# inksci/TRPO

Measured on AMD Instinct MI355X. Metric: TRPO updates/sec (10-iter CG + linesearch) at N states; FVP GB/s vs HBM peak, higher is better.
Workload: dtype fp32 (f16x3 split); 1 GPU; C4: 8M states, obs 128, 256x256 tanh MLP, 18 actions; full update = discount+standardise+pg+10 CG+shs FVP+line search+final losses; n_states=8000000, obs_dim=128, n_actions=18, num_params=103442, cg_iters=10, parallelism=dp1 (row shards, RCCL all-reduce of [P] FVP/grad + loss scalars)

## Files before the change

### trpo_amd/csrc/engine.cpp

```cpp
#include "../../include/trpo_engine.h"
#include "abi_util.h"
#include "common.h"
#include "kernels.h"

#include <hip/hip_runtime.h>
#include <rccl/rccl.h>

#include <algorithm>
#include <cmath>
#include <cstddef>
#include <cstdio>
#include <cstdlib>
#include <cstring>
#include <map>
#include <memory>
#include <stdexcept>
#include <string>
#include <type_traits>
#include <vector>

using namespace trpo;

using namespace trpo_abi;

// ... 1542 lines not shown
        a.am_a0 = am_ds(1);
        Scope sp(this, "pg_bwdwg_l1");
        launch_rbwd0(a, stream);
        check_launch();
        continue;
      }
      RowGemmArgs a = row_args(w[l], wp[l]);
      a.nseg = 1;
      a.seg[0] = bwd_seg(l, kW, DS[l], am_ds(l));
      a.epi = RowEpi::kPgBwd;
      a.ea.H = H[l];
      a.ea.out0 = DS[l - 1];
      a.ea.amax0 = am_ds(l - 1);
      a.ea.ldo = wp[l];
      Scope sp(this, "pg_bwd", l);
      launch_rowgemm(a, stream);
      check_launch();
    }
    for (int l = r0f ? 1 : 0; l < (have_ds ? L - 1 : L); ++l)
      wgrad_layer(l, 1, WSeg{act_in(l), DS[l], wp[l], wp[l + 1], l == 0 ? am_x() : nullptr, am_ds(l)}, WSeg{}, 0,
                  nullptr, "pg_wgrad");
    reduce_grad(g, nullptr);
  }

  void fvp(const float* v, float* out, const int* skip, int* defer = nullptr) {
    if (defer) *defer = 0;
    reprepare_if_path_changed();
    prepare();
    cache.rd_written();
    cache.slabs_written();
    if (use_fused16()) {
      fvp_fused16(v, out, skip, defer && !multi_rank() && cg_fused_reduce_ok(P) ? defer : nullptr);
      return;
    }
    if (use_fused()) {
      fvp_fused(v, out, skip);
      return;
    }
    if (use_chain()) {
      fvp_chain(v, out, skip);
      return;
    }
    {
      PackArgs pa = pack_args(WF, &WB, 1);
      launch_pack(pa, v, 1, skip, stream);
      check_launch();
    }
    ensure_w3();
    const bool gs = gauss();
    split_parts(false, true, false, !gs, cur_set(), skip, "split_v");
    am_reset(am_rh(0), L);
    am_reset(am_rd(0), L);
    const bool tail = use_tail();
    const int Lf = tail ? L - 1 : L;
    int l_first = 0;
    const bool rh1p = use_rh1_planes();
    if (use_rfwd01()) {
      {
        Scope sp(this, "fvp_rfwd_img");
        launch_rfwd01_img(theta, v, offW[0], offW[1], w[0], am_v(0), am_w(1), am_v(1), rf_img, skip, stream);
        check_launch();
      }
      Rfwd01Args ra{};
      ra.n = n;
      ra.obs = w[0];
      ra.ldh = wp[1];
      ra.ldz = wp[2];
      ra.Xh = Xh;
      ra.Xl = Xl;
      ra.x_mpad = x_mpad;
      ra.eX = pl_e;
      ra.H1 = H[1];
      ra.c0 = v + offb[0];
      ra.c1 = v + offb[1];
      ra.V0 = v + offW[0];
      ra.RH1 = RH[1];
      ra.RZ2 = RH[2];
      ra.img = rf_img;
      ra.am_v0 = am_v(0);
      ra.am_w1 = am_w(1);
      ra.am_v1 = am_v(1);
      ra.am_rh1 = am_rh(1);
      ra.am_rz2 = am_rh(2);
      if (rh1p) ra.e_rh1 = pl_e + 2;
      ra.skip = skip;
      Scope sp(this, "fvp_rfwd01");
      launch_rfwd01(ra, num_cus, stream);
      check_launch();
      l_first = 2;
    }
    for (int l = l_first; l < Lf; ++l) {
      RowGemmArgs a = row_args(w[l + 1], wp[l + 1]);
      if (l == 0) {
        a.nseg = 1;
        a.seg[0] = fwd_seg(0, kV, X, am_x(), cur_set());
        if (planes_l0()) attach_x_planes(a.seg[0], V0b);
      } else {
        a.nseg = 2;
        a.seg[0] = fwd_seg(l, kW, RH[l], am_rh(l), cur_set());
        a.seg[1] = fwd_seg(l, kV, H[l], nullptr, cur_set());
      }
      a.skip = skip;
      a.ea.bias = v + offb[l];
      a.ea.ldo = wp[l + 1];
      if (l < L - 1) {
        a.epi = (tail && l == L - 2) ? RowEpi::kRZ : RowEpi::kRHidden;
        a.ea.H = H[l + 1];
        a.ea.out0 = RH[l + 1];
        a.ea.amax0 = am_rh(l + 1);
      } else {
        a.epi = gs ? RowEpi::kGaussRHead : RowEpi::kRHead;
        a.ea.P = Pm;
        a.ea.logstd = gs ? logstd_of(theta) : nullptr;
        a.ea.out0 = RD[L - 1];
        a.ea.amax0 = am_rd(L - 1);
        a.ea.invN = 1.0 / (double)n_global;
      }
      Scope sp(this, "fvp_rfwd", l);
      launch_rowgemm(a, stream);
      check_launch();
    }
    if (tail) {
      const int l = L - 1;
      TailPackArgs tp{};
      tp.theta = theta;
      tp.v = v;
      tp.off_w = offW[l];
      tp.a = w[l];
      tp.b = w[l + 1];
      tp.am_w = am_w(l);
      tp.am_v = am_v(l);
      tp.out = tail_planes;
      TailArgs ta{};
      ta.rows = (int)n;
      ta.a = w[l];
      ta.b = w[l + 1];
      ta.apad = wp[l];
      ta.bpad = wp[l + 1];
      ta.RH = RH[l];
      ta.rz = 1;
      ta.H = H[l];
      ta.P = Pm;
      ta.DL = D[l];
      ta.c = v + offb[l];
      ta.WV16 = tail_planes;
      ta.WT16 = WB3[l];
      ta.VT16 = WB3[l] + 3 * plane3_b(l);
      ta.bplane = (int64_t)plane3_b(l);
      ta.am_rh = am_rh(l);
      ta.am_d = am_d(l);
      ta.am_w = am_w(l);
      ta.am_v = am_v(l);
      ta.am_out = am_rd(l - 1);
      ta.RDout = RD[l - 1];
      ta.invN = 1.0 / (double)n_global;
      ta.dst = slab_dst(l);
      ta.skip = skip;
      Scope sp(this, "fvp_tail", l);
      launch_tail_pack(tp, stream);
      launch_fvp_tail(ta, stream);
      check_launch();
    }
    const bool r0f = use_rbwd0() && Lf - 1 >= 1;
    for (int l = Lf - 1; l >= 1; --l) {
      if (l == 1 && r0f && gs) {
        RBwd0Args a = rbwd0_args(skip);
        a.nseg = 1;
        a.A0 = RD[1];
        a.am_a0 = am_rd(1);
        Scope sp(this, "fvp_rbwdwg_l1");
        launch_rbwd0(a, stream);
        check_launch();
        continue;
      }
      if (gs) {
        RowGemmArgs a = row_args(w[l], wp[l]);
        a.nseg = 1;
        a.seg[0] = bwd_seg(l, kW, RD[l], am_rd(l));
        a.skip = skip;
        a.epi = RowEpi::kPgBwd;
        a.ea.H = H[l];
        a.ea.out0 = RD[l - 1];
        a.ea.amax0 = am_rd(l - 1);
        a.ea.ldo = wp[l];
        Scope sp(this, "fvp_rbwd", l);
        launch_rowgemm(a, stream);
        check_launch();
        continue;
      }
      if (l == 1 && r0f) {
        RBwd0Args a = rbwd0_args(skip);
        a.nseg = 2;
        a.A0 = RD[1];
        a.A1 = D[1];
        if (cache.d1_plane) {
          a.A1h = D1h;
          a.a1_mpad = cache.d1_mpad;
          a.eA1p = pl_e + 1;
          if (cache.d1_tiled) a.eA1t = eD1t;
        }
        a.am_a0 = am_rd(1);
        a.am_a1 = am_d(1);
        a.E = E[0];
        a.RH = RH[1];
        if (rh1p) a.RHp = rh1_planes();
        Scope sp(this, "fvp_rbwdwg_l1");
        launch_rbwd0(a, stream);
        check_launch();
        continue;
      }
      RowGemmArgs a = row_args(w[l], wp[l]);
      a.nseg = 2;
      a.seg[0] = bwd_seg(l, kW, RD[l], am_rd(l));
      a.seg[1] = bwd_seg(l, kV, D[l], am_d(l));
      a.skip = skip;
      a.epi = RowEpi::kRBwd;
      a.ea.H = H[l];
      a.ea.E = E[l - 1];
      a.ea.RH = RH[l];
      a.ea.out0 = RD[l - 1];
      a.ea.amax0 = am_rd(l - 1);
      a.ea.ldo = wp[l];
      Scope sp(this, "fvp_rbwd", l);
      launch_rowgemm(a, stream);
      check_launch();
    }
    if (gs) {
      for (int l = r0f ? 1 : 0; l < L; ++l)
        wgrad_layer(l, 1, WSeg{act_in(l), RD[l], wp[l], wp[l + 1], l == 0 ? am_x() : nullptr, am_rd(l)}, WSeg{}, 0, skip,
                    "fvp_wgrad");
      reduce_grad(out, skip, 0, v + (P - w[L]));
      return;
    }
    fvp_wgrads(r0f ? 1 : 0, Lf, skip, rh1p);
    reduce_grad(out, skip);
  }

  ChainArgs chain_args(const ImageSet& is, const float* v, const int* skip) const {
    ChainArgs ca{};
    ca.n = (int)n;
    ca.L = L;
    for (int l = 0; l <= L; ++l) {
      ca.w[l] = w[l];
      ca.ld[l] = wp[l];
    }
    ca.X = X;
    for (int l = 0; l < L; ++l) {
      ca.H[l] = H[l];
      ca.RH[l] = RH[l];
      ca.D[l] = D[l];
      ca.E[l] = E[l];
      ca.RD[l] = RD[l];
      ca.offb[l] = offb[l];
    }
    ca.P = Pm;
    ca.v = v;
    ca.img = is.img;
    ca.tab = is.tab;
    ca.nchunks = is.nchunks;
    ca.invN = 1.0 / (double)n_global;
    ca.skip = skip;
    return ca;
  }
  void chain_w_images(const float* v) {
    if (cache.chain_w_valid) return;
    Scope sp(this, "fvp_img_w");
    launch_chain_img(chain_set.jobs, theta, v, 0, nullptr, stream);
    check_launch();
    cache.chain_w_valid = true;
  }
  void chain_images(const float* v, const int* skip) {
    chain_w_images(v);
    Scope sp(this, "fvp_img_v");
    launch_chain_img(chain_set.jobs, theta, v, 1, skip, stream);
    check_launch();
  }

  void fvp_fused(const float* v, float* out, const int* skip) {
    chain_images(v, skip);
    const int variant = g_options.fused == 1 ? 1 : 2;
    const int rb = fused_fvp_states_per_group(variant);
    FusedArgs fa{};
    fa.c = chain_args(chain_set, v, skip);
    fa.slab = slab;
    fa.slab_stride = slab_stride;
    for (int l = 0; l < L; ++l) fa.offW[l] = offW[l];
    fa.ngroups = (int)((n + rb - 1) / rb);
    const int per_cu = variant == 2 ? 2 : 1;
    const int grid =
        (int)std::max<int64_t>(1, std::min<int64_t>({(int64_t)fa.ngroups, (int64_t)S, (int64_t)num_cus * per_cu}));
    {
      Scope sp(this, "fvp_fused");
      launch_fvp_fused(fa, grid, variant, stream);
      check_launch();
    }
    reduce_grad(out, skip, grid);
  }

  Fused16Args fused16_args(const float* v, const int* skip, int& grid) {
    const int rb = fused16_states_per_group();
    Fused16Args fa{};
    fa.f.c = chain_args(f16_set, v, skip);
    fa.f.slab = slab;
    fa.f.slab_stride = slab_stride;
    for (int l = 0; l < L; ++l) fa.f.offW[l] = offW[l];
    fa.f.ngroups = (int)((n + rb - 1) / rb);
// ... 1373 lines not shown
```

### trpo_amd/csrc/kernels.h

```cpp
#pragma once
#include <hip/hip_runtime.h>
#include <cstdint>

namespace trpo {

struct Options {
  int split_mfma;
  int split_wg;
  int chain;
  int split_f16;
  int split_min_k;
  int graphs;
  int tail;
  int fused;
  int low_seg;
  int planes;
  int rbwd0;
  int hbwd2;
  int head_fwd;
  int splits;
  int pg_splits;
  int ls_fused;
  int cg_fuse_reduce;
  int cg_p_img;
  int rfwd01;
  int fwd01;
  int rh1_planes;
  int rbwd0_bdma;
};

constexpr int kAmaxSub = 256, kAmaxStride = 32, kAmaxSlot = kAmaxSub * kAmaxStride;

__host__ __device__ inline int f16_scale_exp(float m) {
  if (!(m > 0.0f) || !(m < 3.0e38f)) return 0;
  int q = 0;
  (void)frexpf(m, &q);
  int e = 12 - q;
  return e < -100 ? -100 : (e > 100 ? 100 : e);
}
extern Options g_options;
int* option_slot(const char* name);

struct GemmSeg {
  const float* A;
  const float* B;
  int lda, ldb, K;
  const uint16_t* B3 = nullptr;
  int ldk = 0, plane = 0;
  const unsigned* amaxA = nullptr;
  const unsigned* amaxB = nullptr;
  const uint16_t* Ah = nullptr;
  const uint16_t* Al = nullptr;
  int ldp = 0, mpad = 0;
  const int* eAp = nullptr;
  const uint16_t* Bb = nullptr;
};

enum class RowEpi : int {
  kTanh = 0,
  kRHidden = 1,
  kPrepBwd = 2,
  kPgBwd = 3,
  kRBwd = 4,
  kPrepHead = 5,
  kLossHead = 6,
  kRHead = 7,
  kRelu = 8,
  kReluBwd = 9,
  kPrepBwdE = 10,
  kRZ = 11,
  kGaussPrepHead = 12,
  kGaussLossHead = 13,
  kGaussRHead = 14,
};
constexpr int kMaxHeadTiles = 4;
constexpr bool epi_is_gauss(int e) { return e >= (int)RowEpi::kGaussPrepHead && e <= (int)RowEpi::kGaussRHead; }
constexpr bool epi_is_head(int e) {
  return (e >= (int)RowEpi::kPrepHead && e <= (int)RowEpi::kRHead) || epi_is_gauss(e);
}

struct RowEpiArgs {
  const float* bias;
  const float* H;
  const float* E;
  const float* RH;
  float* out0;
  float* out1;
  float* out2;
  int ldo;
  const float* P;
  const float* old;
  const int* act;
  const float* adv;
  double* rowterms;
  double invN;
  unsigned* amax0 = nullptr;
  unsigned* amax1 = nullptr;
  unsigned* amax2 = nullptr;
  const float* actf = nullptr;
  const float* logstd = nullptr;
  const float* logstd0 = nullptr;
};

struct RowGemmArgs {
  int M, N, Npad;
  int nseg;
  GemmSeg seg[2];
  const int* skip;
  RowEpi epi;
  RowEpiArgs ea;
  int f16 = 0;
  int low_seg = 0;
};

void launch_rowgemm(const RowGemmArgs& a, hipStream_t s);
void launch_rowgemm_planes(const RowGemmArgs& a, hipStream_t s);
void launch_split_planes(const float* A, int M, int Mpad, int K, int lda, uint16_t* hi, uint16_t* lo, int ldp,
                         const unsigned* amax, int* e_out, hipStream_t s);
void launch_block_planes(const uint16_t* src, int P, int R, int ld, uint16_t* dst, hipStream_t s);
bool rowgemm_uses_split(int Npad, RowEpi epi);

struct SplitJob {
  const float* B;
  uint16_t* B3;
  int K, Npad, ldb, ldk;
  const unsigned* amax = nullptr;
};
constexpr int kMaxSplitJobs = 16;
struct SplitArgs {
  int n;
  SplitJob job[kMaxSplitJobs];
  int f16 = 0;
};
void launch_split_b(const SplitArgs& a, const int* skip, hipStream_t s);

struct SlabDst {
  int splits = 0, rows_per_split = 0;
  float* slab = nullptr;
  int64_t slab_stride = 0;
  int64_t off_w = 0, off_b = 0;
};

struct PairPlane {
  const unsigned* hi = nullptr;
  const unsigned* lo = nullptr;
  const int* e = nullptr;
};
constexpr int kPairLd = 256;
constexpr int64_t pair_plane_dwords(int64_t rows) { return (rows + 1) / 2 * kPairLd; }

struct WSeg {
  const float* A;
  const float* B;
  int lda, ldb;
  const unsigned* amaxA = nullptr;
  const unsigned* amaxB = nullptr;
  PairPlane Ap{};
};

struct WGradArgs {
  int rows;
  int Ma, Nb;
  int Mpad, Npad;
  int nseg;
  WSeg seg[2];
  int colsum_seg;
  SlabDst dst;
  const int* skip;
  int f16 = 0;
  int low_seg = 0;
};

void launch_wgrad(const WGradArgs& a, hipStream_t s);

struct LayerPack {
  int64_t off_w;
  int a, b, apad, bpad;
  float* WF;
  float* WB;
  unsigned* amax = nullptr;
};
// ... 95 lines not shown
  void* dst;
};
struct GatherArgs {
  GatherWide wide[3];
  GatherScalar scalar[2];
  int nwide, nscalar;
  int64_t n_sub, stride;
  int64_t first;
  const float* whole_src;
  float* whole_dst;
  int64_t whole_n;
};
void launch_gather_feed(const GatherArgs& a, int num_cus, hipStream_t s);

size_t discount_workspace_bytes(int64_t n);
void launch_discount(const double* x, const uint8_t* starts, int64_t n, double gamma, double* out,
                     void* workspace, hipStream_t s);
void launch_adv_center_partials(const double* returns, const double* baseline, double* adv,
                                int64_t n, double* partials, hipStream_t s);
void launch_sum_finish(const double* partials, double* out, hipStream_t s);
void launch_adv_sq_partials(const double* adv, int64_t n, const double* global_sum, double inv_n,
                            double* partials, hipStream_t s);
void launch_adv_normalize(double* adv, float* adv32, int64_t n, const double* global_sum,
                          const double* global_sq, double inv_n, hipStream_t s);

size_t gae_workspace_bytes(int64_t n);
void launch_gae(const double* rewards, const double* values, const uint8_t* starts, const double* tail_values,
                int64_t n, double gamma, double lambda, double* adv, double* returns, void* workspace,
                hipStream_t s);

}

namespace trpo {
struct ChainArgs {
  int n, L;
  int w[kMaxLayers + 1];
  int ld[kMaxLayers + 1];
  const float* X;
  const float* H[kMaxLayers];
  float* RH[kMaxLayers];
  const float* P;
  const float* D[kMaxLayers];
  const float* E[kMaxLayers];
  float* RD[kMaxLayers];
  const float* v;
  int64_t offb[kMaxLayers];
  const void* img;
  const int* tab;
  int nchunks;
  double invN;
  const int* skip;
};

struct ChainImgJob {
  int64_t src_off, dst_off;
  int K, O, ldw, trans, kc, otp, which, pad;
};
constexpr int kMaxChainJobs = 4 * kMaxLayers;
struct ChainImgArgs {
  int n;
  ChainImgJob job[kMaxChainJobs];
  unsigned short* img;
};
int chain_max_tiles(int max_hidden);
void launch_fvp_chain(const ChainArgs& a, int otm, hipStream_t s);
void launch_chain_img(const ChainImgArgs& a, const float* theta, const float* v, int which, const int* skip,
                      hipStream_t s);

struct FusedArgs {
  ChainArgs c;
  float* slab;
  int64_t slab_stride;
  int64_t offW[kMaxLayers];
  int ngroups;
};
bool fused_fvp_eligible(int L, const int* w);
int fused_fvp_states_per_group(int variant);
void launch_fvp_fused(const FusedArgs& a, int grid, int variant, hipStream_t s);

constexpr int kFused16Jobs = 9;
struct Fused16Args {
  FusedArgs f;
  const int* img_e;
  const unsigned* am_x;
  const unsigned* am_d1;
  const unsigned* am_d2;
  const float* DS;
  const unsigned* am_ds2;
  float* D1out;
  float* E1out;
  float* E0out;
  unsigned* am_d1_out;
};
bool fused16_eligible(int L, const int* w);
int fused16_obs_chunks(int obs);
int fused16_states_per_group();
int fused16_groups_per_cu();
void launch_cg_p_img16(const ChainImgArgs& a, const float* r, const float* p_old, float* p_new, int64_t n,
                       UpdScalars* sc, const double* partials2, CGFlags* fl, int it, int* img_e, hipStream_t s);
void launch_fused16_img(const ChainImgArgs& a, const float* theta, const float* v, int which, const int* skip,
                        int* img_e, hipStream_t s);
void launch_fvp_fused16(const Fused16Args& a, int grid, hipStream_t s);
void launch_pg_fused16(const Fused16Args& a, int grid, hipStream_t s);
void launch_prep_pg_fused16(const Fused16Args& a, int grid, hipStream_t s);
struct FwdLoss16Args {
  int64_t n;
  int L = 3;
  int w[4], ld[4];
  const float* X;
  const float* theta;
  int64_t offb[3];
  const void* img;
  const int* tab;
  int nchunks;
  const int* img_e;
  const unsigned* am_x;
  const float* old;
  const int* act;
  const float* adv;
  double* rowterms;
  const int* skip;
  float* H1 = nullptr;
  float* H2 = nullptr;
  float* P = nullptr;
  float* D = nullptr;
  float* DS = nullptr;
  unsigned* am_d = nullptr;
  unsigned* am_ds = nullptr;
  double invN = 0.0;
};
void launch_fwd_loss16(const FwdLoss16Args& a, int num_cus, hipStream_t s);
}

namespace trpo {
constexpr int kTailK = 256;
struct TailArgs {
  int rows, a, b, apad, bpad;
  const float* RH;
  const float* H;
  int rz = 0;
  const float* P;
  const float* DL;
  const float* c;
  const uint16_t* WV16;
  const uint16_t* WT16;
  const uint16_t* VT16;
  int64_t bplane;
  const unsigned *am_rh, *am_d, *am_w, *am_v;
  unsigned* am_out;
  float* RDout;
  double invN;
  SlabDst dst;
  const int* skip;
};
struct TailPackArgs {
  const float* theta;
  const float* v;
  int64_t off_w;
  int a, b;
  const unsigned *am_w, *am_v;
  uint16_t* out;
};
bool tail_eligible(int apad, int bpad);

struct RBwd0Args {
  int rows;
  int K, lda;
  int N, Npad;
  int obs;
  int nseg;
  const float* A0;
  const float* A1;
  const uint16_t* A1h;
  const int* eA1t = nullptr;
  int a1_mpad;
  const int* eA1p;
  const uint16_t* B0;
  const uint16_t* B1;
  int ldk;
  int64_t plane;
  const unsigned *am_a0, *am_b0, *am_a1, *am_b1;
  const float* H;
  const float* E;
  const float* RH;
  PairPlane RHp{};
  const uint16_t* Xh;
  const uint16_t* Xl;
  int x_mpad, x_ldp;
  const int* eX;
  SlabDst dst;
  const int* skip;
  int low_seg = 0;
};
struct HeadBwd2Args {
  int rows;
  int A, Apad;
  int N, Npad;
  const float* WB;
  const float* D2;
  const float* DS2;
  const float* H;
  float* D1;
  float* DS1;
  unsigned* am_d1;
  unsigned* am_ds1;
  uint16_t* D1h = nullptr;
  int d1_mpad = 0;
  int* eD1t = nullptr;
  float* E1 = nullptr;
  SlabDst dst;
};
bool head_bwd2_eligible(int A, int Npad);
struct HeadFwdArgs {
  int64_t rows;
  int A, Apad;
  int K, Kpad;
  const float* H;
  const float* W;
  const float* bias;
  const float* old;
  const int* act;
  const float* adv;
  double* rowterms;
  double invN;
  int prep = 0;
  float* P = nullptr;
  float* D = nullptr;
  float* DS = nullptr;
  unsigned* am_d = nullptr;
  unsigned* am_ds = nullptr;
};
bool head_fwd_eligible(int A, int K);
void launch_head_fwd(const HeadFwdArgs& a, int num_cus, hipStream_t s);
void launch_head_bwd2(const HeadBwd2Args& a, int num_cus, hipStream_t s);
struct Rfwd01Args {
  int64_t n;
  int obs, ldh, ldz;
  const uint16_t *Xh, *Xl;
  int x_mpad;
  const int* eX;
  const float *H1, *c0, *c1;
  const float* V0;
  float *RH1, *RZ2;
  int* e_rh1 = nullptr;
  const uint16_t* img;
  const unsigned *am_v0, *am_w1, *am_v1;
  unsigned *am_rh1, *am_rz2;
  const int* skip;
};
struct Fwd01Args {
  int64_t n;
  int obs;
  const uint16_t *Xh, *Xl;
  int x_mpad;
  const int* eX;
  const float *b0, *b1;
  float *H1, *H2;
  const uint16_t* img;
  const unsigned *am_w0, *am_w1;
};
constexpr bool rfwd01_rows_ok(int64_t x_mpad) { return 4 * x_mpad * 64 < (int64_t(1) << 31); }
static_assert(rfwd01_rows_ok((1 << 23) - 256) && !rfwd01_rows_ok(1 << 23), "rfwd01 / fwd01 row limit");
constexpr bool pair_planes_rows_ok(int64_t x_mpad) { return rfwd01_rows_ok(x_mpad); }
bool fwd01_eligible(int L, const int* w, const int* wp);
size_t fwd01_img_bytes();
void launch_fwd01_img(const float* th, int64_t offW0, int64_t offW1, int obs, const unsigned* am_w0,
                      const unsigned* am_w1, uint16_t* img, hipStream_t s);
void launch_fwd01(const Fwd01Args& a, int num_cus, hipStream_t s);
bool rfwd01_eligible(int L, const int* w, const int* wp);
size_t rfwd01_img_bytes();
void launch_rfwd01_img(const float* theta, const float* v, int64_t offV0, int64_t offW1, int obs,
                       const unsigned* am_v0, const unsigned* am_w1, const unsigned* am_v1, uint16_t* img,
                       const int* skip, hipStream_t s);
void launch_rfwd01(const Rfwd01Args& a, int num_cus, hipStream_t s);
bool rbwd0_eligible(int obs_pad, int x_ldp, int hid_pad, int K);
void launch_rbwd0(const RBwd0Args& a, hipStream_t s);
void launch_tail_pack(const TailPackArgs& p, hipStream_t s);
void launch_fvp_tail(const TailArgs& a, hipStream_t s);
}

namespace trpo {
size_t vf_pos_workspace_bytes(int64_t n);
void launch_vf_features(const float* obs, int obs_dim, int ld_obs, const float* dist, int A, int ld_dist,
                        const uint8_t* starts, int64_t n, int64_t* lastpos, void* ws, float* feat, int Fp,
                        hipStream_t s, const int64_t* step_index = nullptr);
void launch_vf_tail_features(const float* obs, int obs_dim, const float* dist, int A, const int64_t* lengths,
                             int64_t n_paths, float* feat, int Fp, hipStream_t s);
void launch_vf_tail_scatter(const float* pred, const uint8_t* truncated, const int64_t* end_rows, int64_t n_paths,
                            int64_t n, double* tail, hipStream_t s);
struct VFPackArgs {
  int F, H1, H2, H1p, H2p;
  int64_t offW1, offW2;
  float* W1p;
  float* W2p;
  float* W2T;
};
void launch_vf_pack(const VFPackArgs& a, const float* theta, hipStream_t s);
struct VFHeadArgs {
  int64_t n;
  int H2, H2p;
  const float* Z2;
  const float* w3;
  const float* b3;
  int train;
  const float* y;
  float* dout;
// ... 121 lines not shown
```

### trpo_amd/csrc/options.cpp

```cpp
#include "kernels.h"

#include <cstdlib>
#include <cstring>

namespace trpo {
namespace {

struct OptionRow {
  const char* name;
  const char* env;
  int Options::*field;
  int dflt;
};
constexpr OptionRow kOptionRows[] = {
    {"split_mfma", "TRPO_SPLIT_MFMA", &Options::split_mfma, 5},
    {"split_wg", "TRPO_SPLIT_WG", &Options::split_wg, 1},
    {"chain", "TRPO_CHAIN", &Options::chain, 1},
    {"split_f16", "TRPO_SPLIT_F16", &Options::split_f16, 1},
    {"split_min_k", "TRPO_SPLIT_MIN_K", &Options::split_min_k, 0},
    {"graphs", "TRPO_GRAPHS", &Options::graphs, 1},
    {"tail", "TRPO_TAIL", &Options::tail, 1},
    {"fused", "TRPO_FUSED", &Options::fused, 3},
    {"low_seg", "TRPO_LOW_SEG", &Options::low_seg, 14},
    {"planes", "TRPO_PLANES", &Options::planes, 1},
    {"rbwd0", "TRPO_RBWD0", &Options::rbwd0, 1},
    {"hbwd2", "TRPO_HBWD2", &Options::hbwd2, 2},
    {"head_fwd", "TRPO_HEAD_FWD", &Options::head_fwd, 1},
    {"splits", "TRPO_SPLITS", &Options::splits, 0},
    {"pg_splits", "TRPO_PG_SPLITS", &Options::pg_splits, 0},
    {"ls_fused", "TRPO_LS_FUSED", &Options::ls_fused, 1},
    {"cg_fuse_reduce", "TRPO_CG_FUSE_REDUCE", &Options::cg_fuse_reduce, 1},
    {"cg_p_img", "TRPO_CG_P_IMG", &Options::cg_p_img, 1},
    {"rfwd01", "TRPO_RFWD01", &Options::rfwd01, 1},
    {"fwd01", "TRPO_FWD01", &Options::fwd01, 1},
    {"rh1_planes", "TRPO_RH1_PLANES", &Options::rh1_planes, 1},
    {"rbwd0_bdma", "TRPO_RBWD0_BDMA", &Options::rbwd0_bdma, 1},
};
static_assert(sizeof kOptionRows / sizeof kOptionRows[0] == sizeof(Options) / sizeof(int),
              "every field of Options needs a row");

Options options_from_env() {
  Options o{};
  for (const OptionRow& r : kOptionRows) {
    const char* e = std::getenv(r.env);
    o.*r.field = e ? std::atoi(e) : r.dflt;
  }
  return o;
}

}

Options g_options = options_from_env();

int* option_slot(const char* name) {
  for (const OptionRow& r : kOptionRows)
    if (!std::strcmp(name, r.name)) return &(g_options.*r.field);
  return nullptr;
}

}
```

### trpo_amd/csrc/tail.hip

```cpp
#include "split.h"

#include <stdexcept>

namespace trpo {
namespace {

constexpr int TR = 32;
constexpr int NW = 8;
constexpr int SLD = 36;

#ifndef TRPO_TAIL_HEAD64
#define TRPO_TAIL_HEAD64 0
#endif

__device__ __forceinline__ int sw_off(int mat, int plane, int j, int k) {
  return ((mat * 2 + plane) * 32 + j) * kTailK + (((k >> 3) ^ (j & 15)) << 3) + (k & 7);
}

__global__ void __launch_bounds__(NW * 64, 1) fvp_tail_kernel(const TailArgs A) {
  __shared__ __attribute__((aligned(16))) unsigned short sW[2 * 2 * 32 * kTailK];
  __shared__ __attribute__((aligned(16))) unsigned short sX[NW][2 * 2 * 32 * 32];
  __shared__ __attribute__((aligned(16))) float sRD[2][TR][SLD];
  __shared__ __attribute__((aligned(16))) float sD[2][TR][SLD];
  __shared__ __attribute__((aligned(16))) unsigned short sP[2 * 2 * TR * 32];
  __shared__ float sMax[2][NW];
  __shared__ float sBias[NW][64];
  __shared__ float sOut[NW];
  if (A.skip && *A.skip) return;

  const int tid = threadIdx.x, lane = tid & 63, w = tid >> 6;
  const int lr = lane & 31, lh = lane >> 5;
  const int apad = A.apad, bpad = A.bpad, b = A.b;
  const int r0 = blockIdx.x * A.dst.rows_per_split;
  const int r1 = min(A.rows, r0 + A.dst.rows_per_split);
  const int col0 = 32 * w;
  const bool wv = col0 < apad;

  const int eRH = amax_exp(A.am_rh), eD = amax_exp(A.am_d), eW = amax_exp(A.am_w), eV = amax_exp(A.am_v);
  const int eH = f16_scale_exp(1.0f);
  const float sRHf = __builtin_ldexpf(1.0f, eRH), sDf = __builtin_ldexpf(1.0f, eD), sHf = __builtin_ldexpf(1.0f, eH);

  for (int i = tid; i < 2 * 2 * 32 * (kTailK / 8); i += NW * 64) {
    const int c = i % (kTailK / 8), row = i / (kTailK / 8);
    const int j = row & 31;
    *reinterpret_cast<u16x8*>(sW + row * kTailK + ((c ^ (j & 15)) << 3)) =
        *reinterpret_cast<const u16x8*>(A.WV16 + (size_t)row * kTailK + 8 * c);
  }

  f16x8 wt[2][2], vt[2][2];
  {
    const int n = col0 + lr;
    const bool nv = n < apad;
#pragma unroll
    for (int s = 0; s < 2; ++s)
#pragma unroll
      for (int p = 0; p < 2; ++p) {
        const size_t o = (size_t)p * A.bplane + (size_t)(nv ? n : 0) * 32 + 16 * s + 8 * lh;
        const u16x8 x = *reinterpret_cast<const u16x8*>(A.WT16 + o);
        const u16x8 y = *reinterpret_cast<const u16x8*>(A.VT16 + o);
        wt[s][p] = nv ? __builtin_bit_cast(f16x8, x) : f16x8{};
        vt[s][p] = nv ? __builtin_bit_cast(f16x8, y) : f16x8{};
      }
  }
  __syncthreads();

  f32x16 G = f32x16{};
  float bsum = 0.0f;
  float mxo = 0.0f;

  auto desc = [&](const float* p, int t0, int ld) {
    const int nr = max(0, min(TR, r1 - t0));
    return __builtin_amdgcn_make_buffer_rsrc((void*)(p + (size_t)t0 * ld), 0, nr * ld * 4, 0x00020000);
  };
  const int vo_c = wv ? ((4 * lh) * apad + col0 + lr) * 4 : 0x40000000;
  const int hrow0 = ((2 * w) & 3) + 8 * ((2 * w) >> 2) + 4 * lh;
  const int vo_h = lr < bpad ? (hrow0 * bpad + lr) * 4 : 0x40000000;
  auto load_c = [&](int t0, float (&rh)[16], float (&h)[16], float (&pp)[2], float (&dd)[2]) {
    const __amdgpu_buffer_rsrc_t rRH = desc(A.RH, t0, apad), rH = desc(A.H, t0, apad);
#pragma unroll
    for (int i = 0; i < 16; ++i) {
      const int so = ((i & 3) + 8 * (i >> 2)) * apad * 4;
      rh[i] = ldbuf(rRH, vo_c, so);
      h[i] = ldbuf(rH, vo_c, so);
    }
    const __amdgpu_buffer_rsrc_t rP = desc(A.P, t0, bpad), rDL = desc(A.DL, t0, bpad);
#pragma unroll
    for (int q = 0; q < 2; ++q) {
      pp[q] = ldbuf(rP, vo_h, q * bpad * 4);
      dd[q] = ldbuf(rDL, vo_h, q * bpad * 4);
    }
  };

  float cRH[16], cH[16], cP[2], cD[2];
  if (r0 < r1) load_c(r0, cRH, cH, cP, cD);
  int par = 0;
  for (int t0 = r0; t0 < r1; t0 += TR, par ^= 1) {
    float nRH[16], nH[16], nP[2], nD[2];
    if (t0 + TR < r1) load_c(t0 + TR, nRH, nH, nP, nD);
    if (A.rz) {
#pragma unroll
      for (int i = 0; i < 16; ++i) cRH[i] = one_minus_sq(cH[i]) * cRH[i];
    }

    unsigned short* xw = sX[w];
    auto xoff = [](int mat, int plane, int k, int m) {
      return ((mat * 2 + plane) * 32 + k) * 32 + ((((m >> 2) ^ ((k >> 1) & 7))) << 2) + (m & 3);
    };
#pragma unroll
    for (int s2 = 0; s2 < 2; ++s2) {
      f16x8 hi, lo;
#pragma unroll
      for (int mat = 0; mat < 2; ++mat) {
        split8(mat == 0 ? &cRH[8 * s2] : &cH[8 * s2], mat == 0 ? sRHf : sHf, hi, lo);
        const s16x4* hp = reinterpret_cast<const s16x4*>(&hi);
        const s16x4* lp = reinterpret_cast<const s16x4*>(&lo);
#pragma unroll
        for (int half = 0; half < 2; ++half) {
          const int m = 16 * s2 + 8 * half + 4 * lh;
          *reinterpret_cast<s16x4*>(xw + xoff(mat, 0, lr, m)) = hp[half];
          *reinterpret_cast<s16x4*>(xw + xoff(mat, 1, lr, m)) = lp[half];
        }
      }
    }
    {
      const int g4 = lane >> 4, q = (lane >> 2) & 3, pp = lane & 3;
      const int mrow = 16 * (g4 & 1) + 4 * pp;
      f32x16 acc = f32x16{}, accv = f32x16{};
      auto tr8 = [&](int mat, int pl, int s2) {
        s16x8 v;
#pragma unroll
        for (int t = 0; t < 2; ++t) {
          const int k = 16 * s2 + 8 * (g4 >> 1) + 4 * t + q;
          const s16x4 r = __builtin_amdgcn_ds_read_tr16_b64_v4i16(
              (__attribute__((address_space(3))) s16x4*)(xw + xoff(mat, pl, k, mrow)));
#pragma unroll
          for (int e = 0; e < 4; ++e) v[4 * t + e] = r[e];
        }
        return __builtin_bit_cast(f16x8, v);
      };
#pragma unroll
      for (int s2 = 0; s2 < 2; ++s2) {
        const int k = col0 + 16 * s2 + 8 * lh;
        acc = mfma3(tr8(0, 0, s2), tr8(0, 1, s2), *reinterpret_cast<const f16x8*>(sW + sw_off(0, 0, lr, k)),
                    *reinterpret_cast<const f16x8*>(sW + sw_off(0, 1, lr, k)), acc);
        accv = mfma3(tr8(1, 0, s2), tr8(1, 1, s2), *reinterpret_cast<const f16x8*>(sW + sw_off(1, 0, lr, k)),
                     *reinterpret_cast<const f16x8*>(sW + sw_off(1, 1, lr, k)), accv);
      }
      const float f0 = __builtin_ldexpf(1.0f, -(eRH + eW)), f1 = __builtin_ldexpf(1.0f, -(eH + eV));
      float* rzw = reinterpret_cast<float*>(xw);
#pragma unroll
      for (int i = 0; i < 16; ++i) rzw[i * 64 + lane] = acc[i] * f0 + accv[i] * f1;
    }
    lds_barrier();

    float m = 0.0f;
    {
      const int j = lr;
      const bool real = j < b;
      const float cj = A.c[real ? j : 0];
#pragma unroll
      for (int q = 0; q < 2; ++q) {
        const int i = 2 * w + q;
        float zs = 0.0f;
#pragma unroll
        for (int u = 0; u < NW; ++u) zs += reinterpret_cast<const float*>(sX[u])[i * 64 + lane];
        const float z = zs + cj;
#if TRPO_TAIL_HEAD64
        typedef double T;
#else
        typedef float T;
#endif
        const T rz = real ? (T)z : T(0);
        const T pd = real ? (T)cP[q] : T(0);
        const T prz = sum32<TRPO_TAIL_DPP>(pd * rz);
        const T Rp = pd * (rz - prz);
        const T inv = T(1) / (pd + (T)kEps);
        const T Aa = real ? pd * inv : T(0);
        const T B = real ? (T)kEps * inv : T(0);
        const T spB = sum32<TRPO_TAIL_DPP>(pd * B);
        const T sRAB = sum32<TRPO_TAIL_DPP>(Rp * Aa * B);
        const T rd = (T)A.invN * (Rp * (B - spB) + Rp * Aa * Aa + pd * sRAB);
        const float rdf = real ? (float)rd : 0.0f;
        const int row = hrow0 + q;
        sRD[par][row][j] = rdf;
        sD[par][row][j] = real ? cD[q] : 0.0f;
        m = fmaxf(m, fabsf(rdf));
        bsum += rdf;
      }
    }
#pragma unroll
    for (int off = 32; off > 0; off >>= 1) m = fmaxf(m, __shfl_xor(m, off, 64));
    if (lane == 0) sMax[par][w] = m;
    lds_barrier();
    float mt = 0.0f;
#pragma unroll
    for (int u = 0; u < NW; ++u) mt = fmaxf(mt, sMax[par][u]);
    const int eRD = f16_scale_exp(mt);
    const float sRDf = __builtin_ldexpf(1.0f, eRD);

    auto pof = [](int mat, int pl, int row, int col) {
      return ((mat * 2 + pl) * TR + row) * 32 + ((((col >> 3) ^ ((row >> 2) & 3))) << 3) + (col & 7);
    };
    {
      const int row = 4 * w + (lane >> 4), col = 2 * (lane & 15);
#pragma unroll
      for (int mat = 0; mat < 2; ++mat) {
        const float sc = mat == 0 ? sRDf : sDf;
        const float a = (mat == 0 ? sRD[par][row][col] : sD[par][row][col]) * sc;
        const float bb = (mat == 0 ? sRD[par][row][col + 1] : sD[par][row][col + 1]) * sc;
        const u32x2 p = split2(a, bb);
        *reinterpret_cast<unsigned*>(sP + pof(mat, 0, row, col)) = p[0];
        *reinterpret_cast<unsigned*>(sP + pof(mat, 1, row, col)) = p[1];
      }
    }
    lds_barrier();

    f32x16 aRW = f32x16{}, aDV = f32x16{}, aDW = f32x16{};
#pragma unroll
    for (int s = 0; s < 2; ++s) {
      const int col = 16 * s + 8 * lh;
      const f16x8 rh_ = *reinterpret_cast<const f16x8*>(sP + pof(0, 0, lr, col));
      const f16x8 rl_ = *reinterpret_cast<const f16x8*>(sP + pof(0, 1, lr, col));
      const f16x8 dh_ = *reinterpret_cast<const f16x8*>(sP + pof(1, 0, lr, col));
      const f16x8 dl_ = *reinterpret_cast<const f16x8*>(sP + pof(1, 1, lr, col));
      aRW = mfma3(rh_, rl_, wt[s][0], wt[s][1], aRW);
      aDV = mfma3(dh_, dl_, vt[s][0], vt[s][1], aDV);
      aDW = mfma3(dh_, dl_, wt[s][0], wt[s][1], aDW);
    }
    {
      const float fRW = __builtin_ldexpf(1.0f, -(eRD + eW)), fDV = __builtin_ldexpf(1.0f, -(eD + eV));
      const float fDW = __builtin_ldexpf(1.0f, -(eD + eW));
      const __amdgpu_buffer_rsrc_t rOut = desc(A.RDout, t0, apad);
#pragma unroll
      for (int i = 0; i < 16; ++i) {
        const float rdh = aRW[i] * fRW + aDV[i] * fDV;
        const float dh = aDW[i] * fDW;
        const float h = cH[i], rh = cRH[i];
        const float e = -2.0f * dh * h;
        const float o = fmaf(e, rh, rdh * one_minus_sq(h));
        __builtin_amdgcn_raw_buffer_store_b32(__builtin_bit_cast(unsigned, o), rOut, vo_c,
                                              ((i & 3) + 8 * (i >> 2)) * apad * 4, 0);
        mxo = fmaxf(mxo, fabsf(o));
      }
    }
    {
      const int g4 = lane >> 4, q = (lane >> 2) & 3, pp = lane & 3;
      auto trb = [&](int mat, int pl, int s2) {
        s16x8 v;
#pragma unroll
        for (int t = 0; t < 2; ++t) {
          const int row = 16 * s2 + 4 * (g4 >> 1) + 8 * t + q;
          const s16x4 r = __builtin_amdgcn_ds_read_tr16_b64_v4i16(
              (__attribute__((address_space(3))) s16x4*)(sP + pof(mat, pl, row, 16 * (g4 & 1) + 4 * pp)));
#pragma unroll
          for (int e = 0; e < 4; ++e) v[4 * t + e] = r[e];
        }
        return __builtin_bit_cast(f16x8, v);
      };
      f32x16 g0 = f32x16{}, g1 = f32x16{};
#pragma unroll
      for (int s = 0; s < 2; ++s) {
        f16x8 ah, al;
        split8(&cRH[8 * s], sRHf, ah, al);
        g0 = mfma3(ah, al, trb(1, 0, s), trb(1, 1, s), g0);
        split8(&cH[8 * s], sHf, ah, al);
        g1 = mfma3(ah, al, trb(0, 0, s), trb(0, 1, s), g1);
      }
      const float fG0 = __builtin_ldexpf(1.0f, -(eRH + eD)), fG1 = __builtin_ldexpf(1.0f, -(eH + eRD));
#pragma unroll
      for (int i = 0; i < 16; ++i) G[i] += g0[i] * fG0 + g1[i] * fG1;
    }

    if (t0 + TR < r1) {
#pragma unroll
      for (int i = 0; i < 16; ++i) {
        cRH[i] = nRH[i];
        cH[i] = nH[i];
      }
#pragma unroll
      for (int q = 0; q < 2; ++q) {
        cP[q] = nP[q];
        cD[q] = nD[q];
      }
    }
  }

  float* out = A.dst.slab + (size_t)blockIdx.x * A.dst.slab_stride;
  if (lr < b) {
#pragma unroll
    for (int i = 0; i < 16; ++i) {
      const int mrow = col0 + (i & 3) + 8 * (i >> 2) + 4 * lh;
      if (mrow < A.a) out[A.dst.off_w + (int64_t)mrow * b + lr] = G[i];
    }
  }
  sBias[w][lane] = bsum;
#pragma unroll
  for (int off = 32; off > 0; off >>= 1) mxo = fmaxf(mxo, __shfl_xor(mxo, off, 64));
  if (lane == 0) sOut[w] = mxo;
  __syncthreads();
  if (tid < b) {
    float t = 0.0f;
#pragma unroll
    for (int q = 0; q < NW; ++q) t += sBias[q][tid] + sBias[q][tid + 32];
    out[A.dst.off_b + tid] = t;
  }
  if (tid == 0 && A.am_out) {
    float mm = 0.0f;
#pragma unroll
    for (int q = 0; q < NW; ++q) mm = fmaxf(mm, sOut[q]);
    if (mm > 0.0f) atomicMax(A.am_out + (blockIdx.x % kAmaxSub) * kAmaxStride, __float_as_uint(mm));
  }
}

__global__ void __launch_bounds__(256) tail_pack_kernel(const TailPackArgs P) {
  const int mat = blockIdx.y;
  const float* src = (mat == 0 ? P.theta : P.v) + P.off_w;
  const int e = amax_exp(mat == 0 ? P.am_w : P.am_v);
  const float s = __builtin_ldexpf(1.0f, e);
  const int idx = blockIdx.x * 256 + threadIdx.x;
  if (idx >= 32 * kTailK) return;
  const int j = idx / kTailK, k = idx % kTailK;
  const float x = (j < P.b && k < P.a) ? src[(size_t)k * P.b + j] * s : 0.0f;
  unsigned short hh, ll;
  split2_rn(x, hh, ll);
  P.out[((size_t)(mat * 2 + 0) * 32 + j) * kTailK + k] = hh;
  P.out[((size_t)(mat * 2 + 1) * 32 + j) * kTailK + k] = ll;
}

}

bool tail_eligible(int apad, int bpad) {
  return apad > 128 && apad <= kTailK && apad % 32 == 0 && bpad > 16 && bpad <= 32;
}

void launch_tail_pack(const TailPackArgs& p, hipStream_t s) {
  hipLaunchKernelGGL(tail_pack_kernel, dim3((32 * kTailK + 255) / 256, 2), dim3(256), 0, s, p);
}

void launch_fvp_tail(const TailArgs& a, hipStream_t s) {
  if (!tail_eligible(a.apad, a.bpad) || a.b > 32 || a.a > a.apad)
    throw std::runtime_error("fvp_tail: unsupported layer shape");
  if (a.dst.splits <= 0) return;
  if (a.dst.rows_per_split % TR) throw std::runtime_error("fvp_tail: rows_per_split % 32");
  hipLaunchKernelGGL(fvp_tail_kernel, dim3(a.dst.splits), dim3(NW * 64), 0, s, a);
}

}
```

Measured before the change: 2.547 updates/s.

## Add reduced-precision tail FVP variant selected by on-device exponent sampling

```diff
diff --git a/trpo_amd/csrc/engine.cpp b/trpo_amd/csrc/engine.cpp
--- a/trpo_amd/csrc/engine.cpp
+++ b/trpo_amd/csrc/engine.cpp
@@ -1718,6 +1718,7 @@
       ta.am_w = am_w(l);
       ta.am_v = am_v(l);
       ta.am_out = am_rd(l - 1);
+      ta.am_rdl = am_rd(l);
       ta.RDout = RD[l - 1];
       ta.invN = 1.0 / (double)n_global;
       ta.dst = slab_dst(l);
diff --git a/trpo_amd/csrc/kernels.h b/trpo_amd/csrc/kernels.h
--- a/trpo_amd/csrc/kernels.h
+++ b/trpo_amd/csrc/kernels.h
@@ -27,6 +27,7 @@
   int fwd01;
   int rh1_planes;
   int rbwd0_bdma;
+  int tail_form;
 };
 
 constexpr int kAmaxSub = 256, kAmaxStride = 32, kAmaxSlot = kAmaxSub * kAmaxStride;
@@ -428,6 +429,8 @@
   double invN;
   SlabDst dst;
   const int* skip;
+  unsigned* am_rdl = nullptr;
+  int low_seg = 0;
 };
 struct TailPackArgs {
   const float* theta;
diff --git a/trpo_amd/csrc/options.cpp b/trpo_amd/csrc/options.cpp
--- a/trpo_amd/csrc/options.cpp
+++ b/trpo_amd/csrc/options.cpp
@@ -35,6 +35,7 @@
     {"fwd01", "TRPO_FWD01", &Options::fwd01, 1},
     {"rh1_planes", "TRPO_RH1_PLANES", &Options::rh1_planes, 1},
     {"rbwd0_bdma", "TRPO_RBWD0_BDMA", &Options::rbwd0_bdma, 1},
+    {"tail_form", "TRPO_TAIL_FORM", &Options::tail_form, 1},
 };
 static_assert(sizeof kOptionRows / sizeof kOptionRows[0] == sizeof(Options) / sizeof(int),
               "every field of Options needs a row");
diff --git a/trpo_amd/csrc/tail.hip b/trpo_amd/csrc/tail.hip
--- a/trpo_amd/csrc/tail.hip
+++ b/trpo_amd/csrc/tail.hip
@@ -17,6 +17,20 @@
   return ((mat * 2 + plane) * 32 + j) * kTailK + (((k >> 3) ^ (j & 15)) << 3) + (k & 7);
 }
 
+__device__ __forceinline__ bool tail_one(const TailArgs& A, int eRH, int eD, int eW, int eV, int eH) {
+  const int lane = threadIdx.x & 63;
+  float m = 0.0f;
+#pragma unroll
+  for (int i = 0; i < kAmaxSub / 64; ++i) m = fmaxf(m, __uint_as_float(A.am_rdl[(lane + 64 * i) * kAmaxStride]));
+#pragma unroll
+  for (int off = 32; off > 0; off >>= 1) m = fmaxf(m, __shfl_xor(m, off, 64));
+  const int eRD = f16_scale_exp(m), ls = A.low_seg;
+  const bool f = ls > 0 && m > 0.0f && (eD + eV) - (eRD + eW) >= ls && (eD + eRH - 13) - eRD >= ls &&
+                 (eRH + eD) - (eH + eRD) >= ls + 4;
+  return __builtin_amdgcn_readfirstlane(f ? 1 : 0) != 0;
+}
+
+template <bool ONE>
 __global__ void __launch_bounds__(NW * 64, 1) fvp_tail_kernel(const TailArgs A) {
   __shared__ __attribute__((aligned(16))) unsigned short sW[2 * 2 * 32 * kTailK];
   __shared__ __attribute__((aligned(16))) unsigned short sX[NW][2 * 2 * 32 * 32];
@@ -27,7 +41,6 @@
   __shared__ float sBias[NW][64];
   __shared__ float sOut[NW];
   if (A.skip && *A.skip) return;
-
   const int tid = threadIdx.x, lane = tid & 63, w = tid >> 6;
   const int lr = lane & 31, lh = lane >> 5;
   const int apad = A.apad, bpad = A.bpad, b = A.b;
@@ -38,6 +51,7 @@
 
   const int eRH = amax_exp(A.am_rh), eD = amax_exp(A.am_d), eW = amax_exp(A.am_w), eV = amax_exp(A.am_v);
   const int eH = f16_scale_exp(1.0f);
+  if (A.am_rdl && tail_one(A, eRH, eD, eW, eV, eH) != ONE) return;
   const float sRHf = __builtin_ldexpf(1.0f, eRH), sDf = __builtin_ldexpf(1.0f, eD), sHf = __builtin_ldexpf(1.0f, eH);
 
   for (int i = tid; i < 2 * 2 * 32 * (kTailK / 8); i += NW * 64) {
@@ -210,7 +224,7 @@
         const float bb = (mat == 0 ? sRD[par][row][col + 1] : sD[par][row][col + 1]) * sc;
         const u32x2 p = split2(a, bb);
         *reinterpret_cast<unsigned*>(sP + pof(mat, 0, row, col)) = p[0];
-        *reinterpret_cast<unsigned*>(sP + pof(mat, 1, row, col)) = p[1];
+        if (!(ONE && mat == 1)) *reinterpret_cast<unsigned*>(sP + pof(mat, 1, row, col)) = p[1];
       }
     }
     lds_barrier();
@@ -222,10 +236,16 @@
       const f16x8 rh_ = *reinterpret_cast<const f16x8*>(sP + pof(0, 0, lr, col));
       const f16x8 rl_ = *reinterpret_cast<const f16x8*>(sP + pof(0, 1, lr, col));
       const f16x8 dh_ = *reinterpret_cast<const f16x8*>(sP + pof(1, 0, lr, col));
-      const f16x8 dl_ = *reinterpret_cast<const f16x8*>(sP + pof(1, 1, lr, col));
-      aRW = mfma3(rh_, rl_, wt[s][0], wt[s][1], aRW);
-      aDV = mfma3(dh_, dl_, vt[s][0], vt[s][1], aDV);
-      aDW = mfma3(dh_, dl_, wt[s][0], wt[s][1], aDW);
+      if constexpr (ONE) {
+        aRW = mfma3(rh_, rl_, wt[s][0], wt[s][1], aRW);
+        aDV = __builtin_amdgcn_mfma_f32_32x32x16_f16(dh_, vt[s][0], aDV, 0, 0, 0);
+        aDW = __builtin_amdgcn_mfma_f32_32x32x16_f16(dh_, wt[s][0], aDW, 0, 0, 0);
+      } else {
+        const f16x8 dl_ = *reinterpret_cast<const f16x8*>(sP + pof(1, 1, lr, col));
+        aRW = mfma3(rh_, rl_, wt[s][0], wt[s][1], aRW);
+        aDV = mfma3(dh_, dl_, vt[s][0], vt[s][1], aDV);
+        aDW = mfma3(dh_, dl_, wt[s][0], wt[s][1], aDW);
+      }
     }
     {
       const float fRW = __builtin_ldexpf(1.0f, -(eRD + eW)), fDV = __builtin_ldexpf(1.0f, -(eD + eV));
@@ -257,14 +277,34 @@
         }
         return __builtin_bit_cast(f16x8, v);
       };
+      auto own8 = [&](int pl, int s) {
+        s16x8 v;
+#pragma unroll
+        for (int half = 0; half < 2; ++half) {
+          const s16x4 r = *reinterpret_cast<const s16x4*>(xw + xoff(1, pl, lr, 16 * s + 8 * half + 4 * lh));
+#pragma unroll
+          for (int e = 0; e < 4; ++e) v[4 * half + e] = r[e];
+        }
+        return __builtin_bit_cast(f16x8, v);
+      };
       f32x16 g0 = f32x16{}, g1 = f32x16{};
 #pragma unroll
       for (int s = 0; s < 2; ++s) {
-        f16x8 ah, al;
-        split8(&cRH[8 * s], sRHf, ah, al);
-        g0 = mfma3(ah, al, trb(1, 0, s), trb(1, 1, s), g0);
-        split8(&cH[8 * s], sHf, ah, al);
-        g1 = mfma3(ah, al, trb(0, 0, s), trb(0, 1, s), g1);
+        if constexpr (ONE) {
+          u32x4 hh;
+#pragma unroll
+          for (int i = 0; i < 4; ++i)
+            hh[i] = __builtin_bit_cast(unsigned,
+                                       __builtin_amdgcn_cvt_pkrtz(cRH[8 * s + 2 * i] * sRHf, cRH[8 * s + 2 * i + 1] * sRHf));
+          g0 = __builtin_amdgcn_mfma_f32_32x32x16_f16(__builtin_bit_cast(f16x8, hh), trb(1, 0, s), g0, 0, 0, 0);
+          g1 = mfma3(own8(0, s), own8(1, s), trb(0, 0, s), trb(0, 1, s), g1);
+        } else {
+          f16x8 ah, al;
+          split8(&cRH[8 * s], sRHf, ah, al);
+          g0 = mfma3(ah, al, trb(1, 0, s), trb(1, 1, s), g0);
+          split8(&cH[8 * s], sHf, ah, al);
+          g1 = mfma3(ah, al, trb(0, 0, s), trb(0, 1, s), g1);
+        }
       }
       const float fG0 = __builtin_ldexpf(1.0f, -(eRH + eD)), fG1 = __builtin_ldexpf(1.0f, -(eH + eRD));
 #pragma unroll
@@ -327,6 +367,46 @@
   P.out[((size_t)(mat * 2 + 1) * 32 + j) * kTailK + k] = ll;
 }
 
+constexpr int kSampleRows = 32;
+__global__ void __launch_bounds__(256) tail_sample_kernel(const TailArgs A) {
+  __shared__ float sZ[8][32];
+  if (A.skip && *A.skip) return;
+  const int eW = amax_exp(A.am_w), eV = amax_exp(A.am_v);
+  const int tid = threadIdx.x, j = tid & 31, c = tid >> 5, row = blockIdx.x;
+  float zw = 0.0f, zv = 0.0f;
+  if (32 * c < A.apad) {
+    const float* rh = A.RH + (size_t)row * A.apad + 32 * c;
+    const float* h = A.H + (size_t)row * A.apad + 32 * c;
+    auto plane = [&](int mat, int pl, int k) {
+      return __builtin_bit_cast(f16x8, *reinterpret_cast<const u16x8*>(A.WV16 + ((size_t)(mat * 2 + pl) * 32 + j) * kTailK + 32 * c + k));
+    };
+#pragma unroll
+    for (int k = 0; k < 32; k += 8) {
+      const f16x8 wh = plane(0, 0, k), wl = plane(0, 1, k), vh = plane(1, 0, k), vl = plane(1, 1, k);
+#pragma unroll
+      for (int e = 0; e < 8; ++e) {
+        const float hk = h[k + e], rk = A.rz ? one_minus_sq(hk) * rh[k + e] : rh[k + e];
+        zw = fmaf(rk, (float)wh[e] + (float)wl[e], zw);
+        zv = fmaf(hk, (float)vh[e] + (float)vl[e], zv);
+      }
+    }
+  }
+  sZ[c][j] = zw * __builtin_ldexpf(1.0f, -eW) + zv * __builtin_ldexpf(1.0f, -eV);
+  __syncthreads();
+  if (tid >= 64) return;
+  const bool real = j < A.b;
+  float z = A.c[real ? j : 0];
+#pragma unroll
+  for (int u = 0; u < 8; ++u) z += sZ[u][j];
+  const float rz = real ? z : 0.0f, pd = real ? A.P[(size_t)row * A.bpad + j] : 0.0f;
+  const float Rp = pd * (rz - sum32<TRPO_TAIL_DPP>(pd * rz));
+  const float inv = 1.0f / (pd + kEps), Aa = real ? pd * inv : 0.0f, B = real ? kEps * inv : 0.0f;
+  const float spB = sum32<TRPO_TAIL_DPP>(pd * B), sRAB = sum32<TRPO_TAIL_DPP>(Rp * Aa * B);
+  const float rd = (float)A.invN * (Rp * (B - spB) + Rp * Aa * Aa + pd * sRAB);
+  const float m = max32<TRPO_TAIL_DPP>(real ? fabsf(rd) : 0.0f);
+  if (tid == 0 && m > 0.0f) atomicMax(A.am_rdl + (blockIdx.x % kAmaxSub) * kAmaxStride, __float_as_uint(m));
+}
+
 }
 
 bool tail_eligible(int apad, int bpad) {
@@ -342,7 +422,16 @@
     throw std::runtime_error("fvp_tail: unsupported layer shape");
   if (a.dst.splits <= 0) return;
   if (a.dst.rows_per_split % TR) throw std::runtime_error("fvp_tail: rows_per_split % 32");
-  hipLaunchKernelGGL(fvp_tail_kernel, dim3(a.dst.splits), dim3(NW * 64), 0, s, a);
-}
-
-}
+  TailArgs t = a;
+  t.low_seg = g_options.low_seg;
+  const dim3 g(t.dst.splits), b(NW * 64);
+  if (g_options.tail_form != 0 && t.low_seg > 0 && t.am_rdl && t.rows > 0) {
+    hipLaunchKernelGGL(tail_sample_kernel, dim3(t.rows < kSampleRows ? t.rows : kSampleRows), dim3(256), 0, s, t);
+    hipLaunchKernelGGL(fvp_tail_kernel<true>, g, b, 0, s, t);
+  } else {
+    t.am_rdl = nullptr;
+  }
+  hipLaunchKernelGGL(fvp_tail_kernel<false>, g, b, 0, s, t);
+}
+
+}
```

Result: no change. 2.546 updates/s (median of 2 runs) (-0.1%).
